# DannielSilva/MM-VQA

Measured on AMD Instinct MI355X. Metric: samples/sec ROCO-MLM pretrain (resnet152+transformer, bs16/GPU, 224^2, seq32), higher is better.
Workload: dtype f32; 1 GPU; pretrain/roco_train.py MLM-only: resnet152 + transformer(4 layers, 12 heads), num_vis 5, hidden 768, vocab 30522, per-GPU batch 16, 224x224, T=32; fwd + log_softmax/NLL + bwd + grad all-reduce + Adam; dropout on, train-mode BN; random-init weights; global_batch=16, seq_len=32, parallelism=dp1

## Files before the change

### mm-vqa_amd/csrc/igemm.hip

```cpp
#include <string>
#include <type_traits>
#include <vector>

#include "kernels.h"

struct FastDiv {
  uint32_t mul, shr, d;
};
struct GemmAux {
  FastDiv ohw, ow;
  int fast;
  int stagger;
  float* part;
  int ldsc;
  int sk_G;
  int sk_gx, sk_gy;
  int sk_slots;
  float* sk_part;
  unsigned* sk_cnt;
  int tick;
  int xcd;
};

__device__ __forceinline__ int fdiv(int n, const FastDiv& f) {
  return f.d == 1 ? n : (int)(__umulhi((uint32_t)n, f.mul) >> f.shr);
}

__device__ __forceinline__ f32x4 ld4(const float* p) { return *reinterpret_cast<const f32x4*>(p); }

typedef _Float16 f16x4 __attribute__((ext_vector_type(4)));
typedef _Float16 f16x8 __attribute__((ext_vector_type(8)));
typedef short s16x4 __attribute__((ext_vector_type(4)));

__host__ __device__ constexpr int km_ld_h(int R) { return R + (((R / 2) % 64 == 16 || (R / 2) % 64 == 48) ? 0 : 32); }
template <int PREC>
__host__ __device__ constexpr int tile_rowk(int R, int BK) { return PREC == MMVQA_PREC_F16 ? R * (BK + 8) / 2 : R * (BK + 4); }
template <int PREC>
__host__ __device__ constexpr int tile_km(int R, int BK) { return PREC == MMVQA_PREC_F16 ? BK * km_ld_h(R) / 2 : BK * (R + 4); }

template <class F, int... Is>
__device__ __forceinline__ void static_for_impl(F&& f, std::integer_sequence<int, Is...>) {
  (f(std::integral_constant<int, Is>{}), ...);
}
template <int N, class F>
__device__ __forceinline__ void static_for(F&& f) {
  static_for_impl(f, std::make_integer_sequence<int, N>{});
}

#define MAX_TAPS 32
#define SC1_AUX 16
#define SK_PART_MAX 8
#define TRY_RET(x) do { int r_ = (x); if (r_ != MMVQA_OK) return r_; } while (0)

#if !defined(IGEMM_TRACE) && (defined(EXP_SAMETILE) || defined(EXP_NOADVANCE) || defined(EXP_NOBAR) || \
                             defined(EXP_NOLOAD) || defined(EXP_NOSTORE) || defined(EXP_NOSTOREC))
#error "the EXP_* ablation switches produce wrong results by design: tracer builds (-DIGEMM_TRACE, tools/igemm_trace.py) only"
#endif
#ifdef IGEMM_TRACE
__device__ unsigned long long* g_igemm_trace = nullptr;
extern "C" int mmvqa_debug_set_trace(unsigned long long* buf) {
  return hipMemcpyToSymbol(HIP_SYMBOL(g_igemm_trace), &buf, sizeof(buf)) == hipSuccess ? 0 : 1;
}
#define TRACE_WG ((size_t)(blockIdx.z * gridDim.y + blockIdx.y) * gridDim.x + blockIdx.x)
#define TRACE_CAP0 ((size_t)(1 << 22) / 8)
#define TRACE_CAP1 ((size_t)(1 << 20) / 8)
#define TRACE_MARK(i)                                                                              \
  do {                                                                                             \
    if (g_igemm_trace && threadIdx.x == 0 && TRACE_WG < TRACE_CAP0) {                              \
      unsigned long long* t_ = g_igemm_trace + ((size_t)(blockIdx.z * gridDim.y + blockIdx.y) * gridDim.x + blockIdx.x) * 8; \
      t_[i] = __builtin_readcyclecounter();                                                        \
      if ((i) == 0) {                                                                              \
        t_[5] = (unsigned long long)__builtin_amdgcn_s_getreg(4 | (0 << 6) | (31 << 11)) |         \
                ((unsigned long long)__builtin_amdgcn_s_getreg(20 | (0 << 6) | (31 << 11)) << 32); \
        t_[6] = __builtin_amdgcn_s_memrealtime();                                                  \
      }                                                                                            \
      if ((i) == 4) t_[7] = __builtin_amdgcn_s_memrealtime();                                      \
    }                                                                                              \
  } while (0)
#define TRACE_STALL_DECL unsigned long long tr_vm = 0, tr_lgkm = 0, tr_bar = 0;
#define TRACE_STALL_FLUSH()                                                                        \
  do {                                                                                             \
    if (g_igemm_trace && threadIdx.x == 0 && TRACE_WG < TRACE_CAP1) {                              \
      unsigned long long* t_ = g_igemm_trace + (1 << 22) + ((size_t)(blockIdx.z * gridDim.y + blockIdx.y) * gridDim.x + blockIdx.x) * 8; \
      t_[0] = tr_vm; t_[1] = tr_lgkm; t_[2] = tr_bar;                                              \
    }                                                                                              \
  } while (0)
#define TRACE_EPI(i)                                                                               \
  do {                                                                                             \
    if (g_igemm_trace && threadIdx.x == 0 && TRACE_WG < TRACE_CAP1)                                \
      g_igemm_trace[(1 << 22) + ((size_t)(blockIdx.z * gridDim.y + blockIdx.y) * gridDim.x + blockIdx.x) * 8 + 4 + (i)] = __builtin_readcyclecounter(); \
  } while (0)
#else
#define TRACE_MARK(i) do {} while (0)
#define TRACE_EPI(i) do {} while (0)
#define TRACE_STALL_DECL
#define TRACE_STALL_FLUSH() do {} while (0)
#endif

template <int BM, int BN, int NT, class Src>
__device__ __forceinline__ void general_epilogue(const GemmParams& p, int m0, int n0, int tid, float* smem, int slot_seed, Src src) {
  constexpr int CH = BN / 4;
  constexpr int RP = NT / CH;
  constexpr int NPASS = BM / RP;
  const int M = p.M, N = p.N;
  const int c4 = tid % CH, rg = tid / CH;
  const int col = n0 + c4 * 4;
  const bool full = col + 3 < N;
  auto ldv = [&](const float* base, size_t off) __attribute__((always_inline)) {
    f32x4 r = {0, 0, 0, 0};
    if (full && !(off & 3)) r = ld4(base + off);
    else {
#pragma unroll
      for (int j = 0; j < 4; ++j) if (col + j < N) r[j] = base[off + j];
    }
    return r;
  };
  auto stv = [&](float* base, size_t off, f32x4 v) __attribute__((always_inline)) {
    if (full && !(off & 3)) *reinterpret_cast<f32x4*>(base + off) = v;
    else {
#pragma unroll
      for (int j = 0; j < 4; ++j) if (col + j < N) base[off + j] = v[j];
// ... 69 lines not shown
            for (int j = 0; j < 4; ++j) v[j] = (mm[u][j] * mks[j] + mkb[j] > 0.f) ? v[j] : 0.f;
          } else {
#pragma unroll
            for (int j = 0; j < 4; ++j) v[j] *= dsilu_f(mm[u][j] * mks[j] + mkb[j]);
          }
        }
#ifndef EXP_NOSTOREC
        stv(C, (size_t)row * ldc + col, v);
#endif
        if (st1) {
          if (stat_bwd) {
#pragma unroll
            for (int j = 0; j < 4; ++j) { sa[j] += v[j]; sb[j] += v[j] * ((zz[u][j] - mu1[j]) * is1[j]); }
            if (st2) {
#pragma unroll
              for (int j = 0; j < 4; ++j) sc[j] += v[j] * ((zz2[u][j] - mu2[j]) * is2[j]);
            }
          } else {
#pragma unroll
            for (int j = 0; j < 4; ++j) { sa[j] += v[j]; sb[j] += v[j] * v[j]; }
          }
        }
        if (colsum) cs += v;
      }
    }
    TRACE_EPI(1);
    if (st1 || colsum) {
      __syncthreads();
      double* red = reinterpret_cast<double*>(smem);
      float* redf = smem + BN * 6;
      for (int i = tid; i < BN * 3; i += NT) red[i] = 0.0;
      for (int i = tid; i < BN; i += NT) redf[i] = 0.f;
      __syncthreads();
      if (cok) {
        if (st1) {
#pragma unroll
          for (int j = 0; j < 4; ++j) {
            double* d = red + (c4 * 4 + j) * 3;
            atomicAdd(d, (double)sa[j]);
            atomicAdd(d + 1, (double)sb[j]);
            if (st2) atomicAdd(d + 2, (double)sc[j]);
          }
        }
        if (colsum) {
#pragma unroll
          for (int j = 0; j < 4; ++j) atomicAdd(&redf[c4 * 4 + j], cs[j]);
        }
      }
      __syncthreads();
      TRACE_EPI(2);
      if (tid < BN && n0 + tid < N) {
        if (st1) {
          const double* d = red + tid * 3;
          const int slot = slot_seed & ((p.stat_slots > 0 ? p.stat_slots : MMVQA_STAT_SLOTS) - 1);
          double* d1 = st1 + ((size_t)slot * N + n0 + tid) * 2;
          atomicAdd(d1, d[0]);
          atomicAdd(d1 + 1, d[1]);
          if (st2) {
            double* d2 = st2 + ((size_t)slot * N + n0 + tid) * 2;
            atomicAdd(d2, d[0]);
            atomicAdd(d2 + 1, d[2]);
          }
        }
        if (colsum) atomicAdd(&colsum[n0 + tid], redf[tid]);
      }
    }
    }
}

template <int BM, int BN, int BK, int KIND, bool NCHW, int KS, bool PERSIST = false, int PREC = MMVQA_PREC_F32>
__global__ __launch_bounds__(256 * KS, 2) void igemm_kernel(const GemmParams p, const GemmAux x) {
  constexpr int NT = 256 * KS;
  constexpr int WM = BM / 2, WN = BN / 2, TM = WM / 32, TN = WN / 32;
  constexpr bool F16 = (PREC == MMVQA_PREC_F16);
  static_assert(!F16 || (KS == 1 && !PERSIST), "the f16 family has no 8-wave or persistent form");
  constexpr bool PIPE = TM * TN <= 2;
  constexpr int LDK = F16 ? BK + 8 : BK + 4;
  constexpr int KQ = BK / 4;
  constexpr int RSTEP = NT / KQ;
  constexpr int NA = BM / RSTEP, NB = BN / RSTEP;
  constexpr bool A_ROWK = (KIND != KIND_WGRAD);
  constexpr bool B_ROWK = (KIND == KIND_FWD);
  constexpr int LDA_KM = F16 ? km_ld_h(BM) : BM + 4, LDB_KM = F16 ? km_ld_h(BN) : BN + 4;
  constexpr int A_TILE = A_ROWK ? tile_rowk<PREC>(BM, BK) : tile_km<PREC>(BM, BK);
  constexpr int B_TILE = B_ROWK ? tile_rowk<PREC>(BN, BK) : tile_km<PREC>(BN, BK);
  constexpr int A_X4 = BM / 4, A_KSTEP = NT / A_X4, NA_KM = BK / A_KSTEP;
  constexpr int B_X4 = BN / 4, B_KSTEP = NT / B_X4, NB_KM = BK / B_KSTEP;
  constexpr int NAC = A_ROWK ? NA : NA_KM;
  constexpr int NBC = B_ROWK ? NB : NB_KM;

  TRACE_MARK(0);
  TRACE_STALL_DECL
  extern __shared__ __attribute__((aligned(16))) float smem[];
  float* As = smem;
  float* Bs = smem + 2 * A_TILE;
  int* taptab = reinterpret_cast<int*>(smem + 2 * A_TILE + 2 * B_TILE);
  float* ctab = smem + 2 * A_TILE + 2 * B_TILE + MAX_TAPS;

  constexpr bool persistent = PERSIST;
  const int nkt_total = (p.K + BK - 1) / BK;
  __shared__ int sk_last;
  long long sk_it = 0, sk_end = 0;
  unsigned sk_Lg = 0;
  const unsigned long long sk_T = (unsigned long long)x.sk_gx * x.sk_gy * nkt_total;
  if (persistent) {
    const unsigned L = blockIdx.x, G = (unsigned)x.sk_G, per = G >> 3;
    sk_Lg = (x.xcd && L < 8u * per) ? (L & 7u) * per + (L >> 3) : L;
    sk_it = (long long)((unsigned long long)sk_Lg * sk_T / G);
    sk_end = (long long)((unsigned long long)(sk_Lg + 1) * sk_T / G);
  }
  for (bool sk_first = true;; sk_first = false) {
  int tid = threadIdx.x;
  if constexpr (persistent) asm volatile("" : "+v"(tid));
  const int lane = tid & 63, wave = (tid >> 6) & 3, ks = tid >> 8;
  const int li = lane & 31, lh = lane >> 5;
  const int wm0 = (wave >> 1) * WM, wn0 = (wave & 1) * WN;
  int bx = blockIdx.x, by = blockIdx.y, bz = blockIdx.z;
  int sk_tile = 0, sk_k0 = 0, sk_k1 = nkt_total;
  if (persistent) {
    if (sk_it >= sk_end) break;
    sk_tile = (int)(sk_it / nkt_total);
    sk_k0 = (int)(sk_it - (long long)sk_tile * nkt_total);
    sk_k1 = (sk_end - sk_it < (long long)(nkt_total - sk_k0)) ? sk_k0 + (int)(sk_end - sk_it) : nkt_total;
    sk_it += sk_k1 - sk_k0;
    if (x.xcd == 2) { by = sk_tile % x.sk_gy; bx = sk_tile / x.sk_gy; } else { bx = sk_tile % x.sk_gx; by = sk_tile / x.sk_gx; }
    bz = 0;
    if (!sk_first) __syncthreads();
  } else if (x.xcd) {
    const unsigned gx = gridDim.x, gy = gridDim.y;
    const unsigned L = bx + gx * (by + gy * bz), per = (gx * gy * gridDim.z) >> 3;
    const unsigned Lg = L < 8u * per ? (L & 7u) * per + (L >> 3) : L;
    if (x.xcd == 1) {
      bx = (int)(Lg % gx);
      const unsigned r = Lg / gx;
      by = (int)(r % gy);
      bz = (int)(r / gy);
    } else {
      by = (int)(Lg % gy);
      const unsigned r = Lg / gy;
      bx = (int)(r % gx);
      bz = (int)(r / gx);
    }
  }
  const int m0 = by * BM, n0 = bx * BN;
#ifdef EXP_SAMETILE
  const int lm0 = 0, ln0 = 0;
#else
  const int lm0 = m0, ln0 = n0;
#endif

  const int kt_begin = persistent ? sk_k0 : bz * p.ktiles_per_split;
  int kt_end = persistent ? sk_k1 : kt_begin + p.ktiles_per_split;
  if (kt_end > nkt_total) kt_end = nkt_total;
  const int nkt = kt_end - kt_begin;
  const int k_begin = kt_begin * BK;

  const int OHW = p.g_OH * p.g_OW;
  const int taps = p.g_KH * p.g_KW;
  const int s = p.g_stride;

  if (!NCHW && A_ROWK && tid < MAX_TAPS) {
    int t = tid < taps ? tid : 0;
    int kh = t / p.g_KW, kw = t - kh * p.g_KW;
    int off = (KIND == KIND_FWD) ? (kh * p.g_SW + kw) * p.a_ld : -((kh / s) * p.g_SW + (kw / s)) * p.a_ld;
    taptab[tid] = off;
  }
  const int fold_C = A_ROWK ? p.g_Cs : BM;
  if (x.ldsc) {
    const BnFold& f = p.a_fold;
    const bool pub = f.publish && (persistent ? (sk_Lg == 0 && sk_first) : (bx == 0 && by == 0 && bz == 0));
// ... 15 lines not shown
    }
  }
  __syncthreads();

  const int a_kq = (tid % KQ) * 4;
  const int a_r0 = tid / KQ;
  int a_base[NAC];
  uint32_t a_mask[NAC];
  int a_c = 0, a_tap = 0;
  int a_pix[NAC], a_y0[NAC], a_x0[NAC];
  int a_img[NAC];
  f32x4 ac0_i = {1, 1, 1, 1}, ac1_i = {0, 0, 0, 0}, ac2_i = {0, 0, 0, 0};
  const int akm_x4 = tid % A_X4, akm_k0 = tid / A_X4;
  if constexpr (A_ROWK) {
    if (x.fast == 0) {
      int k = k_begin + a_kq;
      if (taps > 1) { a_tap = k / p.g_Cs; a_c = k - a_tap * p.g_Cs; } else { a_c = k; a_tap = (k >= p.g_Cs) ? 1 : 0; }
    }
#pragma unroll
    for (int r = 0; r < NA; ++r) {
      const int row = lm0 + a_r0 + RSTEP * r;
      a_base[r] = 0; a_mask[r] = 0; a_pix[r] = 0; a_y0[r] = -(1 << 24); a_x0[r] = -(1 << 24); a_img[r] = 0;
      if (row < p.M) {
        const int n = fdiv(row, x.ohw), rem = row - n * OHW;
        const int oy = fdiv(rem, x.ow), ox = rem - oy * p.g_OW;
        if (p.gate_hw > 0) a_img[r] = row / p.gate_hw;
        if constexpr (NCHW) {
          a_pix[r] = n; a_y0[r] = oy * s - p.g_pad; a_x0[r] = ox * s - p.g_pad;
        } else if (KIND == KIND_FWD) {
          const int y0 = oy * s - p.g_pad, x0 = ox * s - p.g_pad;
          a_base[r] = ((n * p.g_SH + y0) * p.g_SW + x0) * p.a_ld;
          uint32_t xb = 0;
          for (int kw = 0; kw < p.g_KW; ++kw) xb |= ((unsigned)(x0 + kw) < (unsigned)p.g_SW ? 1u : 0u) << kw;
          uint32_t mk = 0;
          for (int kh = 0; kh < p.g_KH; ++kh) mk |= ((unsigned)(y0 + kh) < (unsigned)p.g_SH ? xb : 0u) << (kh * p.g_KW);
          a_mask[r] = mk;
        } else {
          const int ty = oy + p.g_pad, tx = ox + p.g_pad;
          if (s <= 2) {
            const int sh = s - 1, sm = s - 1;
            const int qy = ty >> sh, ry = ty & sm, qx = tx >> sh, rx = tx & sm;
            a_base[r] = ((n * p.g_SH + qy) * p.g_SW + qx) * p.a_ld;
            uint32_t xb = 0;
            for (int kw = 0; kw < p.g_KW; ++kw)
              xb |= (((kw & sm) == rx && (unsigned)(qx - (kw >> sh)) < (unsigned)p.g_SW) ? 1u : 0u) << kw;
            uint32_t mk = 0;
            for (int kh = 0; kh < p.g_KH; ++kh)
              mk |= (((kh & sm) == ry && (unsigned)(qy - (kh >> sh)) < (unsigned)p.g_SH) ? xb : 0u) << (kh * p.g_KW);
            a_mask[r] = mk;
          } else {
            const int qy = ty / s, ry = ty - qy * s, qx = tx / s, rx = tx - qx * s;
            a_base[r] = ((n * p.g_SH + qy) * p.g_SW + qx) * p.a_ld;
            uint32_t mk = 0;
            for (int t = 0; t < taps; ++t) {
              const int kh = t / p.g_KW, kw = t - kh * p.g_KW;
              const int sy = qy - kh / s, sx = qx - kw / s;
              if ((kh % s) == ry && (kw % s) == rx && sy >= 0 && sy < p.g_SH && sx >= 0 && sx < p.g_SW) mk |= 1u << t;
            }
            a_mask[r] = mk;
          }
        }
      }
    }
  } else {
    const int i = lm0 + akm_x4 * 4;
#pragma unroll
    for (int r = 0; r < NA_KM; ++r) {
      a_base[r] = (k_begin + akm_k0 + A_KSTEP * r) * p.a_ld + i;
      a_mask[r] = (i < p.M) ? 1u : 0u;
    }
    if (p.a_pro != PRO_NONE && i < p.M) {
      if (x.ldsc) {
        ac0_i = *reinterpret_cast<const f32x4*>(&ctab[akm_x4 * 4]);
        ac1_i = *reinterpret_cast<const f32x4*>(&ctab[BM + akm_x4 * 4]);
        ac2_i = *reinterpret_cast<const f32x4*>(&ctab[2 * BM + akm_x4 * 4]);
      } else {
        ac0_i = ld4(p.a_c0 + i); ac1_i = ld4(p.a_c1 + i);
        if (p.a_pro == PRO_DZ) ac2_i = ld4(p.a_c2 + i);
      }
    }
  }

  const int b_kq = (tid % KQ) * 4, b_r0 = tid / KQ;
  const int bkm_x4 = tid % B_X4, bkm_k0 = tid / B_X4;
  int b_base[NBC];
  uint32_t b_ok0[NBC];
  int b_co[NBC], b_tap[NBC];
  f32x4 bc0 = {1, 1, 1, 1}, bc1 = {0, 0, 0, 0};
  int b_kh = 0, b_kw = 0, b_ci = 0;
  int b_dy[4], b_dx[4], b_cc[4];
  bool b_colvalid = true;
  if constexpr (KIND == KIND_FWD) {
#pragma unroll
    for (int r = 0; r < NB; ++r) {
      const int n = ln0 + b_r0 + RSTEP * r;
      b_ok0[r] = n < p.N;
      b_base[r] = (n < p.N ? n : 0) * p.b_ld + b_kq + k_begin;
    }
  } else if constexpr (KIND == KIND_DGRAD) {
    const int n = ln0 + bkm_x4 * 4;
    b_colvalid = n < p.N;
#pragma unroll
    for (int r = 0; r < NB_KM; ++r) {
      int k = k_begin + bkm_k0 + B_KSTEP * r;
      b_tap[r] = 0; b_co[r] = k;
      if (x.fast == 0) {
        if (taps > 1) { b_tap[r] = k / p.g_Cs; b_co[r] = k - b_tap[r] * p.g_Cs; }
        else { b_tap[r] = (k >= p.g_Cs) ? 1 : 0; }
      }
      b_base[r] = n; b_ok0[r] = 1;
    }
  } else {
    const int nn = ln0 + bkm_x4 * 4;
    b_colvalid = nn < p.N;
    if constexpr (!NCHW) {
      int tap = 0;
      if (taps > 1) { tap = nn / p.g_Cs; b_kh = tap / p.g_KW; b_kw = tap - b_kh * p.g_KW; }
      b_ci = nn - tap * p.g_Cs;
      if (p.b_pro != PRO_NONE && b_colvalid) { bc0 = ld4(p.b_c0 + b_ci); bc1 = ld4(p.b_c1 + b_ci); }
    } else {
#pragma unroll
      for (int j = 0; j < 4; ++j) {
        int kk = nn + j;
        int tap = kk / p.g_Cs;
        b_cc[j] = kk - tap * p.g_Cs;
        b_dy[j] = tap / p.g_KW; b_dx[j] = tap - b_dy[j] * p.g_KW;
        if (kk >= p.N) b_dy[j] = -(1 << 24);
      }
    }
#pragma unroll
    for (int r = 0; r < NB_KM; ++r) { b_base[r] = k_begin + bkm_k0 + B_KSTEP * r; b_ok0[r] = 1; }
  }

  struct Stage {
    f32x4 ra[NAC], ra2[NAC], rb[NBC], rb2[NBC];
    uint32_t a_ok, b_ok;
    f32x4 ac0, ac1, ac2;
    int tm[NAC];
    int pm[NBC], tmb[NBC];
  };

  f32x16 acc[TM][TN];
#pragma unroll
  for (int i = 0; i < TM; ++i)
#pragma unroll
    for (int j = 0; j < TN; ++j)
#pragma unroll
      for (int e = 0; e < 16; ++e) acc[i][j][e] = 0.f;

  const int adv_tap = BK / p.g_Cs, adv_c = BK - adv_tap * p.g_Cs;

  auto lds_put = [&](float* tile, int e, f32x4 v) __attribute__((always_inline)) {
    if constexpr (F16) *reinterpret_cast<f16x4*>(reinterpret_cast<_Float16*>(tile) + e) = __builtin_convertvector(v, f16x4);
    else *reinterpret_cast<f32x4*>(&tile[e]) = v;
  };

  auto run = [&](auto APRO_T, auto BPRO_T, auto FAST_T, auto LDSC_T) __attribute__((always_inline)) {
    constexpr int APRO = decltype(APRO_T)::value;
    constexpr int BPRO = decltype(BPRO_T)::value;
    constexpr int FAST = decltype(FAST_T)::value;
    constexpr bool LDSC = decltype(LDSC_T)::value;
    constexpr bool A_TWO = (APRO == PRO_DZ);
    constexpr bool A_AFF = (APRO == PRO_AFFINE_RELU || APRO == PRO_AFFINE_SILU || APRO == PRO_SILU_GATE);
    constexpr bool B_AFF = (BPRO == PRO_AFFINE_RELU || BPRO == PRO_AFFINE_SILU || BPRO == PRO_SILU_GATE);

    constexpr int NLP = 1 + NAC + NBC;
    bool lt_kvalid = false;
    int lt_toff = 0;
    int lt_kh[4], lt_kw[4], lt_c[4];
    auto load_piece = [&](Stage& S, int kt, int i) __attribute__((always_inline)) {
      if (i == 0) {
        S.a_ok = 0; S.b_ok = 0;
        if constexpr (A_ROWK && !NCHW) {
          lt_kvalid = a_tap < taps;
          lt_toff = taptab[lt_kvalid ? a_tap : 0];
          if constexpr (A_AFF || A_TWO) {
            const int cc = lt_kvalid ? a_c : 0;
            S.ac0 = ld4(p.a_c0 + cc); S.ac1 = ld4(p.a_c1 + cc);
            if constexpr (APRO == PRO_DZ) S.ac2 = ld4(p.a_c2 + cc);
          }
        }
        if constexpr (NCHW) {
          S.a_ok = S.b_ok = ~0u;
          if constexpr (A_ROWK) {
#pragma unroll
            for (int j = 0; j < 4; ++j) {
              const int kk = kt * BK + a_kq + j;
              const int tap = kk / p.g_Cs;
              lt_c[j] = kk - tap * p.g_Cs;
              lt_kh[j] = tap / p.g_KW; lt_kw[j] = tap - lt_kh[j] * p.g_KW;
              if (kk >= p.K) lt_kh[j] = -(1 << 24);
            }
          }
        }
      } else if (i <= NAC) {
        const int r = i - 1;
        if constexpr (A_ROWK && !NCHW) {
          const bool ok = lt_kvalid && ((a_mask[r] >> (a_tap & 31)) & 1u);
          const int off = ok ? a_base[r] + lt_toff + a_c : 0;
          S.ra[r] = ld4(p.A + off);
          if constexpr (A_TWO) S.ra2[r] = ld4(p.A2 + off);
          if constexpr (APRO == PRO_SILU_GATE) S.ra2[r] = ld4(p.gate + (ok ? a_img[r] * p.g_Cs + a_c : 0));
          S.a_ok |= (ok ? 1u : 0u) << r;
          if (r == NAC - 1) {
            a_c += adv_c; a_tap += adv_tap;
            const bool wrap = a_c >= p.g_Cs;
            a_c = wrap ? a_c - p.g_Cs : a_c;
            a_tap = wrap ? a_tap + 1 : a_tap;
          }
        } else if constexpr (A_ROWK && NCHW) {
          f32x4 v = {0, 0, 0, 0};
#pragma unroll
          for (int j = 0; j < 4; ++j) {
            const int sy = a_y0[r] + lt_kh[j], sx = a_x0[r] + lt_kw[j];
            if (sy >= 0 && sy < p.g_SH && sx >= 0 && sx < p.g_SW)
              v[j] = p.A[((size_t)(a_pix[r] * p.g_Cs + lt_c[j]) * p.g_SH + sy) * p.g_SW + sx];
          }
          S.ra[r] = v;
        } else {
          const bool ok = a_mask[r] && (kt * BK + akm_k0 + A_KSTEP * r < p.K);
          const int off = ok ? a_base[r] : 0;
          S.ra[r] = ld4(p.A + off);
          if constexpr (A_TWO) S.ra2[r] = ld4(p.A2 + off);
          S.a_ok |= (ok ? 1u : 0u) << r;
          a_base[r] += BK * p.a_ld;
        }
      } else {
        const int r = i - 1 - NAC;
        if constexpr (KIND == KIND_FWD) {
          const int k = kt * BK + b_kq;
          if constexpr (!NCHW) {
            const bool ok = (k < p.K) && b_ok0[r];
            S.rb[r] = ld4(p.B + (ok ? b_base[r] : 0));
            S.b_ok |= (ok ? 1u : 0u) << r;
            b_base[r] += BK;
          } else {
            f32x4 v = {0, 0, 0, 0};
// ... 10 lines not shown
          S.rb[r] = ld4(p.B + off);
          S.b_ok |= (ok ? 1u : 0u) << r;
          b_co[r] += adv_c; b_tap[r] += adv_tap;
          const bool wrap = b_co[r] >= p.g_Cs;
          b_co[r] = wrap ? b_co[r] - p.g_Cs : b_co[r];
          b_tap[r] = wrap ? b_tap[r] + 1 : b_tap[r];
        } else {
          const int m = b_base[r];
          b_base[r] += BK;
          const int n = fdiv(m, x.ohw), rem = m - n * OHW;
          const int oy = fdiv(rem, x.ow), ox = rem - oy * p.g_OW;
          if constexpr (!NCHW) {
            const int sy = oy * s - p.g_pad + b_kh, sx = ox * s - p.g_pad + b_kw;
            const bool ok = (m < p.K) && b_colvalid && sy >= 0 && sy < p.g_SH && sx >= 0 && sx < p.g_SW;
            const int off = ok ? ((n * p.g_SH + sy) * p.g_SW + sx) * p.b_ld + b_ci : 0;
            S.rb[r] = ld4(p.B + off);
            if constexpr (BPRO == PRO_SILU_GATE) S.rb2[r] = ld4(p.gate + (ok ? n * p.g_Cs + b_ci : 0));
            S.b_ok |= (ok ? 1u : 0u) << r;
          } else {
            f32x4 v = {0, 0, 0, 0};
            if (m < p.K) {
#pragma unroll
              for (int j = 0; j < 4; ++j) {
                int sy = oy * s - p.g_pad + b_dy[j], sx = ox * s - p.g_pad + b_dx[j];
                if (sy >= 0 && sy < p.g_SH && sx >= 0 && sx < p.g_SW)
                  v[j] = p.B[((size_t)(n * p.g_Cs + b_cc[j]) * p.g_SH + sy) * p.g_SW + sx];
              }
            }
            S.rb[r] = v;
          }
        }
      }
    };

    auto store_chunk = [&](Stage& S, int buf, int kt, int c) __attribute__((always_inline)) {
      float* as = As + buf * A_TILE;
      float* bs = Bs + buf * B_TILE;
      if (c < NAC) {
        const int r = c;
        f32x4 v = S.ra[r];
        const bool ok = (S.a_ok >> r) & 1u;
        if constexpr (!(NCHW && A_ROWK)) {
          if constexpr (APRO == PRO_AFFINE_RELU) {
#pragma unroll
            for (int j = 0; j < 4; ++j) { float t = v[j] * S.ac0[j] + S.ac1[j]; v[j] = t > 0.f ? t : 0.f; }
          } else if constexpr (APRO == PRO_AFFINE_SILU) {
#pragma unroll
            for (int j = 0; j < 4; ++j) v[j] = silu_f(v[j] * S.ac0[j] + S.ac1[j]);
          } else if constexpr (APRO == PRO_SILU_GATE) {
#pragma unroll
            for (int j = 0; j < 4; ++j) v[j] = silu_f(v[j] * S.ac0[j] + S.ac1[j]) * S.ra2[r][j];
          } else if constexpr (APRO == PRO_DZ) {
#pragma unroll
            for (int j = 0; j < 4; ++j) v[j] = v[j] * S.ac0[j] + S.ra2[r][j] * S.ac1[j] + S.ac2[j];
          }
          const int e0 = A_ROWK ? (kt * BK + a_kq) : (m0 + akm_x4 * 4);
          const int lim = A_ROWK ? p.K : p.M;
#pragma unroll
          for (int j = 0; j < 4; ++j) v[j] = (ok && (e0 + j < lim)) ? v[j] : 0.f;
        }
        if constexpr (A_ROWK) {
          lds_put(as, (a_r0 + RSTEP * r) * LDK + a_kq, v);
        } else {
          lds_put(as, (akm_k0 + A_KSTEP * r) * LDA_KM + akm_x4 * 4, v);
        }
      } else {
        const int r = c - NAC;
        f32x4 v = S.rb[r];
        const bool ok = (S.b_ok >> r) & 1u;
        if constexpr (KIND == KIND_WGRAD && !NCHW && BPRO == PRO_AFFINE_RELU) {
#pragma unroll
          for (int j = 0; j < 4; ++j) { float t = v[j] * bc0[j] + bc1[j]; v[j] = t > 0.f ? t : 0.f; }
        } else if constexpr (KIND == KIND_WGRAD && !NCHW && BPRO == PRO_AFFINE_SILU) {
#pragma unroll
          for (int j = 0; j < 4; ++j) v[j] = silu_f(v[j] * bc0[j] + bc1[j]);
        } else if constexpr (KIND == KIND_WGRAD && !NCHW && BPRO == PRO_SILU_GATE) {
#pragma unroll
          for (int j = 0; j < 4; ++j) v[j] = silu_f(v[j] * bc0[j] + bc1[j]) * S.rb2[r][j];
        }
#pragma unroll
        for (int j = 0; j < 4; ++j) v[j] = ok ? v[j] : 0.f;
        if constexpr (B_ROWK) {
          lds_put(bs, (b_r0 + RSTEP * r) * LDK + b_kq, v);
        } else {
          lds_put(bs, (bkm_k0 + B_KSTEP * r) * LDB_KM + bkm_x4 * 4, v);
        }
      }
    };


    constexpr int BIG = (int)0x80000000;
    __amdgpu_buffer_rsrc_t rA, rA2, rB, rC0, rC1, rC2, rT;
    int f_voffA[NAC], f_voffB[NBC], f_voffT[NBC], f_veB[NBC];
    int f_runT = 0, f_tapw = 0;
    const int f_voffC = a_kq * 4;
    int f_tap = 0, f_c = 0, f_kh = 0, f_kw = 0;
    int f_runA = 0, f_runB = 0;
    int f_sA = 0, f_sB = 0, f_sC = 0;
    const int f_sh = s - 1;
    const int f_maxneg = (KIND == KIND_DGRAD) ? (((p.g_KH - 1) >> f_sh) * p.g_SW + ((p.g_KW - 1) >> f_sh)) * p.a_ld : 0;
    auto bload = [&](__amdgpu_buffer_rsrc_t r, int voff, int soff) __attribute__((always_inline)) {
      return __builtin_bit_cast(f32x4, __builtin_amdgcn_raw_buffer_load_b128(r, voff, soff, 0));
    };
    if constexpr (FAST != 0) {
      constexpr int FLAGS = 0x00020000;
      constexpr int NREC = 0x7FFFF000;
      if constexpr (A_ROWK) {
        const int shift = (KIND == KIND_FWD) ? (p.g_pad * p.g_SW + p.g_pad) * p.a_ld : f_maxneg;
        rA = __builtin_amdgcn_make_buffer_rsrc((void*)(p.A - shift), 0, NREC, FLAGS);
        rA2 = __builtin_amdgcn_make_buffer_rsrc((void*)((A_TWO ? p.A2 : p.A) - shift), 0, NREC, FLAGS);
        const int vshift = (KIND == KIND_FWD) ? shift : 0;
#pragma unroll
        for (int r = 0; r < NAC; ++r) {
          const int off = (a_base[r] + vshift + a_kq) * 4;
          f_voffA[r] = (FAST == 2 || (a_mask[r] & 1u)) ? off : BIG;
        }
        if constexpr ((A_AFF || A_TWO) && !LDSC) {
          rC0 = __builtin_amdgcn_make_buffer_rsrc((void*)p.a_c0, 0, p.g_Cs * 4, FLAGS);
          rC1 = __builtin_amdgcn_make_buffer_rsrc((void*)p.a_c1, 0, p.g_Cs * 4, FLAGS);
          rC2 = __builtin_amdgcn_make_buffer_rsrc((void*)(APRO == PRO_DZ ? p.a_c2 : p.a_c1), 0, p.g_Cs * 4, FLAGS);
        }
        if (k_begin != 0) {
          if (taps > 1) { f_tap = k_begin / p.g_Cs; f_c = k_begin - f_tap * p.g_Cs; } else { f_tap = 0; f_c = k_begin; }
          f_kh = f_tap / p.g_KW; f_kw = f_tap - f_kh * p.g_KW;
        }
      } else {
        rA = __builtin_amdgcn_make_buffer_rsrc((void*)p.A, 0, p.K * p.a_ld * 4, FLAGS);
        rA2 = __builtin_amdgcn_make_buffer_rsrc((void*)(A_TWO ? p.A2 : p.A), 0, p.K * p.a_ld * 4, FLAGS);
#pragma unroll
        for (int r = 0; r < NAC; ++r) f_voffA[r] = a_mask[r] ? a_base[r] * 4 : BIG;
      }
      if constexpr (KIND == KIND_FWD) {
        rB = __builtin_amdgcn_make_buffer_rsrc((void*)p.B, 0, p.N * p.b_ld * 4, FLAGS);
#pragma unroll
        for (int r = 0; r < NBC; ++r) f_voffB[r] = b_ok0[r] ? b_base[r] * 4 : BIG;
      } else if constexpr (KIND == KIND_DGRAD) {
        rB = __builtin_amdgcn_make_buffer_rsrc((void*)p.B, 0, p.g_Cs * p.b_ld * 4, FLAGS);
#pragma unroll
        for (int r = 0; r < NBC; ++r)
          f_voffB[r] = b_colvalid ? ((bkm_k0 + B_KSTEP * r) * p.b_ld + b_base[r]) * 4 : BIG;
      } else if constexpr (FAST == 1) {
        rB = __builtin_amdgcn_make_buffer_rsrc((void*)p.B, 0, p.K * p.b_ld * 4, FLAGS);
#pragma unroll
        for (int r = 0; r < NBC; ++r) f_voffB[r] = b_colvalid ? (b_base[r] * p.b_ld + b_ci) * 4 : BIG;
      } else {
        f_tapw = n0 / p.g_Cs;
        const int kh = f_tapw / p.g_KW, kw = f_tapw - kh * p.g_KW;
        rB = __builtin_amdgcn_make_buffer_rsrc((void*)(p.B - (p.g_pad * p.g_SW + p.g_pad) * p.b_ld), 0, NREC, FLAGS);
        rT = __builtin_amdgcn_make_buffer_rsrc((void*)p.pixmask, 0, p.K * 4, FLAGS);
        f_runB = (kh * p.g_SW + kw) * p.b_ld * 4;
#pragma unroll
        for (int r = 0; r < NBC; ++r) {
          f_voffB[r] = b_colvalid ? (b_base[r] * p.b_ld + b_ci) * 4 : BIG;
          f_voffT[r] = b_base[r] * 4;
        }
      }
#pragma unroll
      for (int r = 0; r < NBC; ++r) f_veB[r] = f_voffB[r];
    }
    int f_ve[NAC];
#pragma unroll
    for (int r = 0; r < NAC; ++r) f_ve[r] = (FAST != 0) ? f_voffA[r] : 0;
    auto tload = [&](int voff, int soff) __attribute__((always_inline)) {
      return __builtin_amdgcn_raw_buffer_load_b32(rT, voff, soff, 0);
    };
    auto f_halo = [&](Stage& S) __attribute__((always_inline)) {
      if constexpr (FAST == 2 && KIND == KIND_WGRAD) {
#pragma unroll
        for (int r = 0; r < NBC; ++r) {
          const int t = __builtin_amdgcn_sbfe(S.pm[r], f_tapw, 1);
          S.tmb[r] = t;
          f_veB[r] = (t & f_voffB[r]) | (~t & BIG);
          S.pm[r] = tload(f_voffT[r], f_runT + 2 * BK * 4);
        }
      } else if constexpr (FAST == 2) {
#pragma unroll
        for (int r = 0; r < NAC; ++r) {
          const int t = __builtin_amdgcn_sbfe((int)a_mask[r], f_tap & 31, 1);
          S.tm[r] = t;
          f_ve[r] = (t & f_voffA[r]) | (~t & BIG);
        }
      }
    };
    auto f_scalars = [&](Stage& S) __attribute__((always_inline)) {
      if constexpr (A_ROWK) {
        const bool live = f_tap < taps;
        const int toff = (KIND == KIND_FWD) ? (f_kh * p.g_SW + f_kw) * p.a_ld
                                            : f_maxneg - ((f_kh >> f_sh) * p.g_SW + (f_kw >> f_sh)) * p.a_ld;
        f_sA = live ? (toff + f_c) * 4 : BIG;
        f_sC = live ? f_c * 4 : BIG;
        if constexpr (KIND == KIND_DGRAD) f_sB = live ? (f_c * p.b_ld + f_tap * p.b_tapstride) * 4 : BIG;
        else f_sB = f_runB;
        if constexpr ((A_AFF || A_TWO) && LDSC) {
          const float* cp = ctab + f_c + a_kq;
          S.ac0 = *reinterpret_cast<const f32x4*>(cp); S.ac1 = *reinterpret_cast<const f32x4*>(cp + fold_C);
          if constexpr (APRO == PRO_DZ) S.ac2 = *reinterpret_cast<const f32x4*>(cp + 2 * fold_C);
        } else if constexpr (A_AFF || A_TWO) {
          S.ac0 = bload(rC0, f_voffC, f_sC); S.ac1 = bload(rC1, f_voffC, f_sC);
          if constexpr (APRO == PRO_DZ) S.ac2 = bload(rC2, f_voffC, f_sC);
        }
      } else {
        f_sA = f_runA; f_sB = f_runB;
      }
    };
    auto f_chunk = [&](Stage& S, int i) __attribute__((always_inline)) {
      if (i < NAC) {
        S.ra[i] = bload(rA, f_ve[i], f_sA);
        if constexpr (A_TWO) S.ra2[i] = bload(rA2, f_ve[i], f_sA);
      } else {
        S.rb[i - NAC] = bload(rB, f_veB[i - NAC], f_sB);
      }
    };
    auto f_advance = [&]() __attribute__((always_inline)) {
#ifdef EXP_NOADVANCE
      return;
#endif
      if constexpr (A_ROWK) {
        f_c += BK;
        if (f_c >= p.g_Cs) {
          f_c = 0; ++f_tap; ++f_kw;
          if (f_kw == p.g_KW) { f_kw = 0; ++f_kh; }
        }
        f_runB += BK * 4;
      } else {
        f_runA += BK * p.a_ld * 4;
        f_runB += BK * p.b_ld * 4;
        f_runT += BK * 4;
      }
    };
    auto fload_piece = [&](Stage& S, int i) __attribute__((always_inline)) {
      if (i == 0) { f_halo(S); f_scalars(S); }
      else f_chunk(S, i - 1);
      if (i == NLP - 1) f_advance();
    };
    auto fstore_chunk = [&](Stage& S, int buf, int c) __attribute__((always_inline)) {
      float* as = As + buf * A_TILE;
      float* bs = Bs + buf * B_TILE;
      typedef float f32x2 __attribute__((ext_vector_type(2)));
      if (c < NAC) {
        const int r = c;
        f32x4 v = S.ra[r];
        if constexpr (APRO == PRO_AFFINE_RELU) {
          const f32x2 lo = __builtin_elementwise_fma(v.xy, S.ac0.xy, S.ac1.xy), hi = __builtin_elementwise_fma(v.zw, S.ac0.zw, S.ac1.zw);
          if constexpr (FAST == 2 && A_ROWK) {
            const float lim = __builtin_bit_cast(float, S.tm[r] & 0x7f800000);
            v[0] = __builtin_amdgcn_fmed3f(lo[0], 0.f, lim); v[1] = __builtin_amdgcn_fmed3f(lo[1], 0.f, lim);
            v[2] = __builtin_amdgcn_fmed3f(hi[0], 0.f, lim); v[3] = __builtin_amdgcn_fmed3f(hi[1], 0.f, lim);
          } else {
            v[0] = fmaxf(lo[0], 0.f); v[1] = fmaxf(lo[1], 0.f); v[2] = fmaxf(hi[0], 0.f); v[3] = fmaxf(hi[1], 0.f);
          }
        } else if constexpr (APRO == PRO_DZ) {
          const f32x4 z = S.ra2[r];
          f32x2 lo = __builtin_elementwise_fma(z.xy, S.ac1.xy, S.ac2.xy), hi = __builtin_elementwise_fma(z.zw, S.ac1.zw, S.ac2.zw);
          lo = __builtin_elementwise_fma(v.xy, S.ac0.xy, lo); hi = __builtin_elementwise_fma(v.zw, S.ac0.zw, hi);
          v[0] = lo[0]; v[1] = lo[1]; v[2] = hi[0]; v[3] = hi[1];
          if constexpr (FAST == 2 && A_ROWK) {
            typedef int i32x4 __attribute__((ext_vector_type(4)));
            const int tmask = S.tm[r];
            const i32x4 vi = __builtin_bit_cast(i32x4, v) & i32x4{tmask, tmask, tmask, tmask};
            v = __builtin_bit_cast(f32x4, vi);
          }
        }
        if constexpr (A_ROWK) {
          lds_put(as, (a_r0 + RSTEP * r) * LDK + a_kq, v);
        } else {
          lds_put(as, (akm_k0 + A_KSTEP * r) * LDA_KM + akm_x4 * 4, v);
        }
      } else {
        const int r = c - NAC;
        f32x4 v = S.rb[r];
        if constexpr (KIND == KIND_WGRAD && BPRO == PRO_AFFINE_RELU) {
          const f32x2 lo = __builtin_elementwise_fma(v.xy, bc0.xy, bc1.xy), hi = __builtin_elementwise_fma(v.zw, bc0.zw, bc1.zw);
          if constexpr (FAST == 2) {
            const float lim = __builtin_bit_cast(float, S.tmb[r] & 0x7f800000);
            v[0] = __builtin_amdgcn_fmed3f(lo[0], 0.f, lim); v[1] = __builtin_amdgcn_fmed3f(lo[1], 0.f, lim);
            v[2] = __builtin_amdgcn_fmed3f(hi[0], 0.f, lim); v[3] = __builtin_amdgcn_fmed3f(hi[1], 0.f, lim);
          } else {
            v[0] = fmaxf(lo[0], 0.f); v[1] = fmaxf(lo[1], 0.f); v[2] = fmaxf(hi[0], 0.f); v[3] = fmaxf(hi[1], 0.f);
          }
        }
        if constexpr (B_ROWK) {
          lds_put(bs, (b_r0 + RSTEP * r) * LDK + b_kq, v);
        } else {
          lds_put(bs, (bkm_k0 + B_KSTEP * r) * LDB_KM + bkm_x4 * 4, v);
        }
      }
    };
    auto LP = [&](Stage& S, int kt, int i) __attribute__((always_inline)) {
      if constexpr (FAST != 0) fload_piece(S, i); else load_piece(S, kt, i);
    };
    auto SC = [&](Stage& S, int buf, int kt, int c) __attribute__((always_inline)) {
      if constexpr (FAST != 0) fstore_chunk(S, buf, c); else store_chunk(S, buf, kt, c);
    };
    auto LT = [&](Stage& S, int kt) __attribute__((always_inline)) {
#pragma unroll
      for (int i = 0; i < NLP; ++i) LP(S, kt, i);
    };

    auto read_frags = [&](const float* as, const float* bs, int kg, f32x4 (&fa)[TM], f32x4 (&fb)[TN]) __attribute__((always_inline)) {
#pragma unroll
      for (int i = 0; i < TM; ++i) {
        if constexpr (A_ROWK) {
          fa[i] = *reinterpret_cast<const f32x4*>(&as[(wm0 + i * 32 + li) * LDK + kg * 8 + lh * 4]);
        } else {
#pragma unroll
          for (int j = 0; j < 4; ++j) fa[i][j] = as[(kg * 8 + lh * 4 + j) * LDA_KM + wm0 + i * 32 + li];
        }
      }
#pragma unroll
      for (int i = 0; i < TN; ++i) {
        if constexpr (B_ROWK) {
          fb[i] = *reinterpret_cast<const f32x4*>(&bs[(wn0 + i * 32 + li) * LDK + kg * 8 + lh * 4]);
        } else {
#pragma unroll
          for (int j = 0; j < 4; ++j) fb[i][j] = bs[(kg * 8 + lh * 4 + j) * LDB_KM + wn0 + i * 32 + li];
        }
      }
    };

    constexpr int NC = NAC + NBC;
    constexpr int NKG = BK / 8 / KS;

    TRACE_MARK(1);
    Stage S0, S1;
    S0.a_ok = S0.b_ok = S1.a_ok = S1.b_ok = 0;
    S0.ac0 = S1.ac0 = ac0_i; S0.ac1 = S1.ac1 = ac1_i; S0.ac2 = S1.ac2 = ac2_i;

    if constexpr (FAST == 2 && KIND == KIND_WGRAD) {
#pragma unroll
      for (int r = 0; r < NBC; ++r) { S0.pm[r] = tload(f_voffT[r], 0); S1.pm[r] = tload(f_voffT[r], BK * 4); }
    }
    if (nkt > 0) {
      LT(S0, kt_begin);
      if constexpr (PIPE) LT(S1, kt_begin + 1);
#pragma unroll
      for (int c = 0; c < NC; ++c) SC(S0, 0, kt_begin, c);
      if constexpr (FAST != 0 && PIPE && !F16) f_halo(S0);
    }
    __builtin_amdgcn_s_waitcnt(0x0F70);
    __syncthreads();
    TRACE_MARK(2);

    if constexpr (F16) {
      auto frag = [&](const float* tile, int rowk, int ldkm, int r0, int st) __attribute__((always_inline)) {
        const _Float16* t = reinterpret_cast<const _Float16*>(tile);
        if (rowk) return *reinterpret_cast<const f16x8*>(t + (r0 + li) * LDK + st * 16 + lh * 8);
        const int g = lane >> 4, q = (lane >> 2) & 3, pp = lane & 3;
        const _Float16* b = t + (st * 16 + (g >> 1) * 8 + q) * ldkm + r0 + (g & 1) * 16 + 4 * pp;
        typedef __attribute__((address_space(3))) s16x4 lds_s16x4;
        const f16x4 lo = __builtin_bit_cast(f16x4, __builtin_amdgcn_ds_read_tr16_b64_v4i16((lds_s16x4*)(b)));
        const f16x4 hi = __builtin_bit_cast(f16x4, __builtin_amdgcn_ds_read_tr16_b64_v4i16((lds_s16x4*)(b + 4 * ldkm)));
        return __builtin_shufflevector(lo, hi, 0, 1, 2, 3, 4, 5, 6, 7);
      };
      auto body16 = [&](int t, Stage& Sload, Stage& Sstore) __attribute__((always_inline)) {
        const int buf = t & 1;
        LT(Sload, kt_begin + t + (PIPE ? 2 : 1));
        const float* as = As + buf * A_TILE;
        const float* bs = Bs + buf * B_TILE;
#pragma unroll
        for (int st = 0; st < BK / 16; ++st) {
          f16x8 fa[TM], fb[TN];
#pragma unroll
          for (int i = 0; i < TM; ++i) fa[i] = frag(as, A_ROWK, LDA_KM, wm0 + i * 32, st);
#pragma unroll
          for (int i = 0; i < TN; ++i) fb[i] = frag(bs, B_ROWK, LDB_KM, wn0 + i * 32, st);
#pragma unroll
          for (int a = 0; a < TM; ++a)
#pragma unroll
            for (int b = 0; b < TN; ++b)
              acc[a][b] = __builtin_amdgcn_mfma_f32_32x32x16_f16(fa[a], fb[b], acc[a][b], 0, 0, 0);
        }
#pragma unroll
        for (int c = 0; c < NC; ++c) SC(Sstore, buf ^ 1, kt_begin + t + 1, c);
        __syncthreads();
      };
      if constexpr (PIPE) {
        int t = 0;
        for (; t + 1 < nkt; t += 2) {
          body16(t, S0, S1);
          body16(t + 1, S1, S0);
        }
        if (t < nkt) body16(t, S0, S1);
      } else {
        for (int t = 0; t < nkt; ++t) body16(t, S0, S0);
      }
    } else if constexpr (PIPE) {
      f32x4 fa[2][TM], fb[2][TN];
      read_frags(As, Bs, ks, fa[0], fb[0]);
      constexpr int MPG = 4 * TM * TN;
      constexpr int NS = NKG * MPG;
      constexpr int SB = NS - MPG;
      constexpr int L0 = 1;
      constexpr int LSTR = (NS - 2) / NLP > 0 ? (NS - 2) / NLP : 1;
      constexpr int ST0 = LSTR >= 2 ? L0 + 1 : L0 + NLP;
// ... 353 lines not shown

  if (p.epi_mode == EPI_TAP_BWD) {
    const int act = p.act, HW = p.tap_HW, ldc = p.c_ld;
    const float inv_hw = 1.0f / (float)HW;
    const float* dv = p.tap_dv;
    float* C = p.C;
#pragma unroll 1
    for (int ps = 0; ps < NPASS; ++ps) {
      const int rl = rg + ps * RP, row = m0 + rl;
      if (row >= M || col >= N) break;
      const int img = row / HW;
      f32x4 v = *reinterpret_cast<const f32x4*>(&ctile[rl * LDC + c4 * 4]);
      const f32x4 g = ldv(dv, (size_t)img * N + col);
#pragma unroll
      for (int j = 0; j < 4; ++j) v[j] = g[j] * inv_hw * act_bwd(act, v[j]);
      stv(C, (size_t)row * ldc + col, v);
    }
    TRACE_MARK(4);
    return;
  }

  general_epilogue<BM, BN, NT>(p, m0, n0, tid, smem, persistent ? by + bx * 7 : (int)(blockIdx.y + blockIdx.x * 7 + blockIdx.z * 3),
                               [&](int rl, int cq) __attribute__((always_inline)) {
                                 return *reinterpret_cast<const f32x4*>(&ctile[rl * LDC + cq * 4]);
                               });
  TRACE_MARK(4);
  if (!persistent) break;
  }
}

constexpr int FOLD_MAX_FLOATS = 3072;
constexpr int SK_MAX = 8;

__global__ __launch_bounds__(256) void splitk_finish_kernel(const GemmParams p, const float* __restrict__ part,
                                                            int nsplit) {
  constexpr int BM = 64, BN = 64;
  __shared__ double smem_d[BN * 3 + BN / 2 + 2];
  const int tid = threadIdx.x, m0 = blockIdx.y * BM, n0 = blockIdx.x * BN;
  const int M = p.M, N = p.N;
  const size_t MN = (size_t)M * N;
  general_epilogue<BM, BN, 256>(p, m0, n0, tid, reinterpret_cast<float*>(smem_d), (int)(blockIdx.y + blockIdx.x * 7),
                                [&](int rl, int cq) __attribute__((always_inline)) {
                                  f32x4 v = {0, 0, 0, 0};
                                  const int row = m0 + rl, col = n0 + cq * 4;
                                  if (row < M && col < N) {
                                    const size_t off = (size_t)row * N + col;
                                    if (col + 3 < N && !(off & 3)) {
                                      f32x4 t[SK_MAX];
#pragma unroll
                                      for (int s = 0; s < SK_MAX; ++s)
                                        t[s] = s < nsplit ? ld4(part + s * MN + off) : f32x4{0, 0, 0, 0};
#pragma unroll
                                      for (int s = 0; s < SK_MAX; ++s) v += t[s];
                                    } else {
                                      for (int s = 0; s < nsplit; ++s)
#pragma unroll
                                        for (int j = 0; j < 4; ++j)
                                          if (col + j < N) v[j] += part[s * MN + off + j];
                                    }
                                  }
                                  return v;
                                });
}

static FastDiv make_fastdiv(int d) {
  FastDiv f;
  f.d = (uint32_t)d;
  if (d <= 1) { f.mul = 0; f.shr = 0; f.d = 1; return f; }
  int lg = 31;
  while (lg > 0 && !((uint32_t)d >> lg)) --lg;
  if (d & (d - 1)) ++lg;
  const int pw = 31 + lg;
  const uint64_t m = ((1ull << pw) + (uint64_t)d - 1) / (uint64_t)d;
  f.mul = (uint32_t)m;
  f.shr = (uint32_t)(pw - 32);
  return f;
}

template <int BM, int BN, int BK, int KIND, bool NCHW, int KS = 1, int PREC = MMVQA_PREC_F32>
static int launch_cfg(GemmParams p, hipStream_t stream) {
  constexpr bool A_ROWK = (KIND != KIND_WGRAD);
  constexpr bool B_ROWK = (KIND == KIND_FWD);
  constexpr int A_TILE = A_ROWK ? tile_rowk<PREC>(BM, BK) : tile_km<PREC>(BM, BK);
  constexpr int B_TILE = B_ROWK ? tile_rowk<PREC>(BN, BK) : tile_km<PREC>(BN, BK);
  constexpr size_t tile_floats = (size_t)(2 * A_TILE + 2 * B_TILE + MAX_TAPS);
  constexpr size_t epi_floats = (size_t)BM * (BN + 4) + 8 * BN;
  constexpr size_t smem_max = (tile_floats + FOLD_MAX_FLOATS > epi_floats ? tile_floats + FOLD_MAX_FLOATS : epi_floats) * sizeof(float);
  static int attr_dev_mask = 0;
  int dev = 0;
  (void)hipGetDevice(&dev);
  if (!(attr_dev_mask >> (dev & 31) & 1)) {
    HIP_CHECK_RET(hipFuncSetAttribute((const void*)igemm_kernel<BM, BN, BK, KIND, NCHW, KS, false, PREC>,
                                      hipFuncAttributeMaxDynamicSharedMemorySize, (int)smem_max));
    attr_dev_mask |= 1 << (dev & 31);
  }
  GemmAux x;
  x.ohw = make_fastdiv(p.g_OH * p.g_OW);
  x.ow = make_fastdiv(p.g_OW);
  x.fast = 0;
  static const int stagger_on = getenv("MMVQA_IGEMM_NOSTAGGER") ? 0 : 1;
  x.stagger = stagger_on;
  x.part = (KIND != KIND_WGRAD && !NCHW && p.splitk > 1 && !p.c_atomic) ? p.sk_ws : nullptr;
  if (!NCHW && (p.K % BK == 0 || (KIND == KIND_WGRAD && p.pixmask)) && !p.gate && !getenv("MMVQA_IGEMM_GENERAL")) {
    const int taps = p.g_KH * p.g_KW;
    const double lim = 2147483648.0 - 16777216.0;
    if (KIND != KIND_WGRAD) {
      const bool pro_ok = (KIND == KIND_FWD) ? (p.a_pro == PRO_NONE || p.a_pro == PRO_AFFINE_RELU)
                                             : (p.a_pro == PRO_NONE || p.a_pro == PRO_DZ);
      const double a_bytes = (KIND == KIND_FWD) ? (double)p.M * p.g_stride * p.g_stride * p.a_ld * 4.0 + (double)(p.g_SW + 2) * p.g_KH * p.a_ld * 4.0
                                                : (double)p.M * p.a_ld * 4.0;
      const double b_bytes = (KIND == KIND_FWD) ? (double)p.N * p.b_ld * 4.0 : (double)p.g_Cs * p.b_ld * 4.0;
      if (pro_ok && p.b_pro == PRO_NONE && p.g_Cs % BK == 0 && p.g_stride <= 2 && a_bytes < lim && b_bytes < lim &&
          (KIND == KIND_FWD || p.N % 4 == 0))
        x.fast = (taps > 1 || (KIND == KIND_DGRAD && p.g_stride > 1)) ? 2 : 1;
    } else {
      const bool pro_ok = (p.a_pro == PRO_NONE || p.a_pro == PRO_DZ) && (p.b_pro == PRO_NONE || p.b_pro == PRO_AFFINE_RELU);
      if (pro_ok && taps == 1 && p.K % BK == 0 && p.g_stride == 1 && p.g_pad == 0 && p.M % 4 == 0 && p.N % 4 == 0 &&
          (double)p.K * p.a_ld * 4.0 < lim && (double)p.K * p.b_ld * 4.0 < lim)
        x.fast = 1;
      else if (pro_ok && taps > 1 && taps <= 32 && p.pixmask && p.g_stride == 1 && p.g_OH == p.g_SH && p.g_OW == p.g_SW &&
               2 * p.g_pad == p.g_KH - 1 && p.g_KH == p.g_KW && BM == 64 && BN == 64 && p.g_Cs % BN == 0 && p.M % 4 == 0 &&
               (double)p.K * p.a_ld * 4.0 < lim && (double)(p.K + (double)p.g_SW * p.g_KH) * p.b_ld * 4.0 < lim)
        x.fast = 2;
    }
  }
  x.ldsc = 0;
  size_t fold_floats = 0;
  if (p.a_fold.stat) {
    const int ncoef = p.a_fold.bwd ? 3 : 2;
    const size_t need = A_ROWK ? (size_t)ncoef * p.g_Cs : (size_t)3 * BM;
    const bool pro_ok = p.a_fold.bwd ? p.a_pro == PRO_DZ : p.a_pro == PRO_AFFINE_RELU;
    if (pro_ok && need <= FOLD_MAX_FLOATS && (KIND == KIND_WGRAD || x.fast != 0)) {
      x.ldsc = 1;
      fold_floats = need;
    } else {
      const BnFold f = p.a_fold;
      const int C = A_ROWK ? p.g_Cs : p.M;
      if (!f.publish || !f.out0 || !f.out1 || !f.out2)
        return mmvqa_set_error(MMVQA_ERR_ARG, "igemm: this launch cannot fold its BatchNorm coefficients in the kernel and has nowhere to publish them");
      if (f.bwd)
        TRY_RET(k_bn_coef_bwd(stream, f.stat, C, f.count, f.gamma, f.mean, f.invstd, 1, f.out0, f.out1, f.out2, f.dgamma, f.dbeta));
      else
        TRY_RET(k_bn_coef_fwd_keep(stream, f.stat, C, f.count, f.eps, f.gamma, f.beta, f.run_mean, f.run_var, f.nbt, f.keep,
                                   f.reps, 1, f.out0, f.out1, f.out2, f.out3));
      p.a_c0 = f.out0; p.a_c1 = f.out1; p.a_c2 = f.out2;
      p.a_fold.stat = nullptr;
    }
  }
  const size_t smem = ((tile_floats + fold_floats > epi_floats ? tile_floats + fold_floats : epi_floats)) * sizeof(float);
  dim3 grid((p.N + BN - 1) / BN, (p.M + BM - 1) / BM, p.splitk);
  x.sk_G = 0; x.sk_gx = (int)grid.x; x.sk_gy = (int)grid.y; x.sk_slots = 0; x.sk_part = nullptr; x.sk_cnt = nullptr; x.tick = 0;
  static const bool finish_form = getenv("MMVQA_SK_FINISH") != nullptr;
  if (x.part && !finish_form && p.sk_cnt && p.splitk <= SK_PART_MAX && p.epi_mode == EPI_PLAIN) {
    const long long tiles = (long long)grid.x * grid.y;
    if (tiles <= p.sk_cnt_n && tiles * p.splitk * (long long)(BM * BN) <= p.sk_ws_floats) {
      x.tick = 1; x.part = nullptr; x.sk_slots = p.splitk; x.sk_part = p.sk_ws; x.sk_cnt = p.sk_cnt;
    }
  }
  if (p.persist > 0 && PREC == MMVQA_PREC_F32 && !NCHW && BM == 64 && BN == 64 && p.epi_mode == EPI_PLAIN && !x.part && p.splitk == 1) {
    const long long tiles = (long long)grid.x * grid.y, nkt = (p.K + BK - 1) / BK, T = tiles * nkt;
    long long G = p.persist < T ? p.persist : T;
    bool ok = G >= 8;
    if (ok && !p.c_atomic) {
      const long long per = T / G;
      const long long slots = (nkt + per - 1) / per + 1;
      ok = slots <= SK_PART_MAX && p.sk_ws && p.sk_cnt && tiles <= p.sk_cnt_n &&
           tiles * slots * (long long)(BM * BN) <= p.sk_ws_floats;
// ... 277 lines not shown
```

Before: 663.4 samples/s.

## Store DGRAD B tile transposed in LDS for vectorized fragment reads

For f32 dgrad kernels, the B operand tile is now written to shared memory in a row-by-k layout instead of k-major. Thread-to-element mapping changes so each thread gathers consecutive k values, buffers them in registers, and writes them transposed. The MFMA fragment reads can then use single 16-byte vector loads instead of four scalar LDS reads. The costs are extra register staging, strided transposed LDS writes with possible bank conflicts, and a different global load coalescing pattern.

Result: no change. 668.5 samples/s (median of 6 runs) (+0.8%).

```diff
diff --git a/mm-vqa_amd/csrc/igemm.hip b/mm-vqa_amd/csrc/igemm.hip
--- a/mm-vqa_amd/csrc/igemm.hip
+++ b/mm-vqa_amd/csrc/igemm.hip
@@ -37,6 +37,11 @@
 __host__ __device__ constexpr int tile_rowk(int R, int BK) { return PREC == MMVQA_PREC_F16 ? R * (BK + 8) / 2 : R * (BK + 4); }
 template <int PREC>
 __host__ __device__ constexpr int tile_km(int R, int BK) { return PREC == MMVQA_PREC_F16 ? BK * km_ld_h(R) / 2 : BK * (R + 4); }
+template <int PREC, int KIND>
+__host__ __device__ constexpr bool b_transposed() { return PREC != MMVQA_PREC_F16 && KIND == KIND_DGRAD; }
+
+__device__ __forceinline__ int km_lane_x4(int tid, int X4) { return ((tid >> 3) & 7) + 8 * ((tid >> 6) % (X4 / 8)); }
+__device__ __forceinline__ int km_lane_kb(int tid, int X4) { return (tid & 7) + 8 * ((tid >> 6) / (X4 / 8)); }
 
 template <class F, int... Is>
 __device__ __forceinline__ void static_for_impl(F&& f, std::integer_sequence<int, Is...>) {
@@ -272,10 +277,12 @@
   constexpr bool A_ROWK = (KIND != KIND_WGRAD);
   constexpr bool B_ROWK = (KIND == KIND_FWD);
   constexpr int LDA_KM = F16 ? km_ld_h(BM) : BM + 4, LDB_KM = F16 ? km_ld_h(BN) : BN + 4;
+  constexpr bool B_TR = b_transposed<PREC, KIND>();
   constexpr int A_TILE = A_ROWK ? tile_rowk<PREC>(BM, BK) : tile_km<PREC>(BM, BK);
-  constexpr int B_TILE = B_ROWK ? tile_rowk<PREC>(BN, BK) : tile_km<PREC>(BN, BK);
+  constexpr int B_TILE = (B_ROWK || B_TR) ? tile_rowk<PREC>(BN, BK) : tile_km<PREC>(BN, BK);
   constexpr int A_X4 = BM / 4, A_KSTEP = NT / A_X4, NA_KM = BK / A_KSTEP;
-  constexpr int B_X4 = BN / 4, B_KSTEP = NT / B_X4, NB_KM = BK / B_KSTEP;
+  constexpr int B_X4 = BN / 4, B_KSTEP = NT / B_X4, NB_KM = BK / B_KSTEP, B_KR = B_TR ? 1 : B_KSTEP;
+  static_assert(!B_TR || ((NB_KM == 2 || NB_KM == 4) && B_X4 % 8 == 0), "transposed B block shape");
   constexpr int NAC = A_ROWK ? NA : NA_KM;
   constexpr int NBC = B_ROWK ? NB : NB_KM;
 
@@ -457,7 +464,8 @@
   }
 
   const int b_kq = (tid % KQ) * 4, b_r0 = tid / KQ;
-  const int bkm_x4 = tid % B_X4, bkm_k0 = tid / B_X4;
+  const int bkm_x4 = B_TR ? km_lane_x4(tid, B_X4) : tid % B_X4;
+  const int bkm_k0 = B_TR ? km_lane_kb(tid, B_X4) * NB_KM : tid / B_X4;
   int b_base[NBC];
   uint32_t b_ok0[NBC];
   int b_co[NBC], b_tap[NBC];
@@ -477,7 +485,7 @@
     b_colvalid = n < p.N;
 #pragma unroll
     for (int r = 0; r < NB_KM; ++r) {
-      int k = k_begin + bkm_k0 + B_KSTEP * r;
+      int k = k_begin + bkm_k0 + B_KR * r;
       b_tap[r] = 0; b_co[r] = k;
       if (x.fast == 0) {
         if (taps > 1) { b_tap[r] = k / p.g_Cs; b_co[r] = k - b_tap[r] * p.g_Cs; }
@@ -504,7 +512,7 @@
       }
     }
 #pragma unroll
-    for (int r = 0; r < NB_KM; ++r) { b_base[r] = k_begin + bkm_k0 + B_KSTEP * r; b_ok0[r] = 1; }
+    for (int r = 0; r < NB_KM; ++r) { b_base[r] = k_begin + bkm_k0 + B_KR * r; b_ok0[r] = 1; }
   }
 
   struct Stage {
@@ -528,6 +536,16 @@
   auto lds_put = [&](float* tile, int e, f32x4 v) __attribute__((always_inline)) {
     if constexpr (F16) *reinterpret_cast<f16x4*>(reinterpret_cast<_Float16*>(tile) + e) = __builtin_convertvector(v, f16x4);
     else *reinterpret_cast<f32x4*>(&tile[e]) = v;
+  };
+  auto put_tr = [&](float* tile, int x4, int k0, const auto& v) __attribute__((always_inline)) {
+    constexpr int NKC = sizeof(v) / sizeof(v[0]);
+    typedef float f32x2 __attribute__((ext_vector_type(2)));
+#pragma unroll
+    for (int j = 0; j < 4; ++j) {
+      float* d = &tile[(4 * x4 + j) * LDK + k0];
+      if constexpr (NKC == 4) *reinterpret_cast<f32x4*>(d) = f32x4{v[0][j], v[1][j], v[2][j], v[3][j]};
+      else *reinterpret_cast<f32x2*>(d) = f32x2{v[0][j], v[1][j]};
+    }
   };
 
   auto run = [&](auto APRO_T, auto BPRO_T, auto FAST_T, auto LDSC_T) __attribute__((always_inline)) {
@@ -704,8 +722,11 @@
         for (int j = 0; j < 4; ++j) v[j] = ok ? v[j] : 0.f;
         if constexpr (B_ROWK) {
           lds_put(bs, (b_r0 + RSTEP * r) * LDK + b_kq, v);
+        } else if constexpr (!B_TR) {
+          lds_put(bs, (bkm_k0 + B_KSTEP * r) * LDB_KM + bkm_x4 * 4, v);
         } else {
-          lds_put(bs, (bkm_k0 + B_KSTEP * r) * LDB_KM + bkm_x4 * 4, v);
+          S.rb[r] = v;
+          if (r == NBC - 1) put_tr(bs, bkm_x4, bkm_k0, S.rb);
         }
       }
     };
@@ -760,7 +781,7 @@
         rB = __builtin_amdgcn_make_buffer_rsrc((void*)p.B, 0, p.g_Cs * p.b_ld * 4, FLAGS);
 #pragma unroll
         for (int r = 0; r < NBC; ++r)
-          f_voffB[r] = b_colvalid ? ((bkm_k0 + B_KSTEP * r) * p.b_ld + b_base[r]) * 4 : BIG;
+          f_voffB[r] = b_colvalid ? ((bkm_k0 + B_KR * r) * p.b_ld + b_base[r]) * 4 : BIG;
       } else if constexpr (FAST == 1) {
         rB = __builtin_amdgcn_make_buffer_rsrc((void*)p.B, 0, p.K * p.b_ld * 4, FLAGS);
 #pragma unroll
@@ -903,8 +924,11 @@
         }
         if constexpr (B_ROWK) {
           lds_put(bs, (b_r0 + RSTEP * r) * LDK + b_kq, v);
+        } else if constexpr (!B_TR) {
+          lds_put(bs, (bkm_k0 + B_KSTEP * r) * LDB_KM + bkm_x4 * 4, v);
         } else {
-          lds_put(bs, (bkm_k0 + B_KSTEP * r) * LDB_KM + bkm_x4 * 4, v);
+          S.rb[r] = v;
+          if (r == NBC - 1) put_tr(bs, bkm_x4, bkm_k0, S.rb);
         }
       }
     };
@@ -931,7 +955,7 @@
       }
 #pragma unroll
       for (int i = 0; i < TN; ++i) {
-        if constexpr (B_ROWK) {
+        if constexpr (B_ROWK || B_TR) {
           fb[i] = *reinterpret_cast<const f32x4*>(&bs[(wn0 + i * 32 + li) * LDK + kg * 8 + lh * 4]);
         } else {
 #pragma unroll
@@ -1451,7 +1475,7 @@
   constexpr bool A_ROWK = (KIND != KIND_WGRAD);
   constexpr bool B_ROWK = (KIND == KIND_FWD);
   constexpr int A_TILE = A_ROWK ? tile_rowk<PREC>(BM, BK) : tile_km<PREC>(BM, BK);
-  constexpr int B_TILE = B_ROWK ? tile_rowk<PREC>(BN, BK) : tile_km<PREC>(BN, BK);
+  constexpr int B_TILE = (B_ROWK || b_transposed<PREC, KIND>()) ? tile_rowk<PREC>(BN, BK) : tile_km<PREC>(BN, BK);
   constexpr size_t tile_floats = (size_t)(2 * A_TILE + 2 * B_TILE + MAX_TAPS);
   constexpr size_t epi_floats = (size_t)BM * (BN + 4) + 8 * BN;
   constexpr size_t smem_max = (tile_floats + FOLD_MAX_FLOATS > epi_floats ? tile_floats + FOLD_MAX_FLOATS : epi_floats) * sizeof(float);
```
